# wtsi-svi/ReadServer

Hardware: AMD Instinct MI355X
Metric: 31-mer backward-search queries/sec on popBWT, counted as (query x shard) backward searches/s (higher is better)
Workload: dtype u64

## Files before the change

### include/rsbwt.h

```cpp
#ifndef RSBWT_H
#define RSBWT_H

#include <stddef.h>
#include <stdint.h>

#ifdef __cplusplus
extern "C" {
#endif

#define RSBWT_OK 0
#define RSBWT_EINVAL (-1)
#define RSBWT_EIO (-2)
#define RSBWT_EFORMAT (-3)
#define RSBWT_ENOMEM (-4)
#define RSBWT_ENODEV (-5)
#define RSBWT_EHIP (-6)
#define RSBWT_ERANGE (-7)
#define RSBWT_ESYS (-8)

#define RSBWT_OPEN_READS 1u
#define RSBWT_OPEN_KTAB_GROUPED 2u
#define RSBWT_KTAB_SHIFT 5
#define RSBWT_KTAB_MASK (0x1Fu << RSBWT_KTAB_SHIFT)
#define RSBWT_KTAB_NONE (31u << RSBWT_KTAB_SHIFT)
// ... 99 lines not shown
size_t rsbwt_1mm_scratch_bytes(const rsbwt_t *h, size_t m, uint32_t k);
int rsbwt_find_intervals_1mm_dev(rsbwt_t *h, const void *d_packed, const void *d_valid, size_t m, uint32_t k,
                                 void *d_lower, void *d_upper, void *d_scratch, void *stream);
size_t rsbwt_hits_1mm_scratch_bytes(const rsbwt_t *h, size_t m, uint32_t k);
int rsbwt_hits_1mm_dev(rsbwt_t *h, const void *d_packed, const void *d_valid, size_t m, uint32_t k, void *d_hits,
                       size_t cap, void *d_total, void *d_scratch, void *stream);
int rsbwt_extract_dev(rsbwt_t *h, const void *d_rows, size_t n, void *d_out, uint32_t stride, void *d_len,
                      void *d_prefix_len, void *stream);

int rsbwt_last_search_ms(rsbwt_t *h, float *ms);
int rsbwt_search_history_ms(rsbwt_t *h, float *ms, size_t cap, size_t *count);
int rsbwt_set_counting(rsbwt_t *h, int on);
int rsbwt_last_search_work(rsbwt_t *h, uint64_t *lf_steps, uint64_t *occ_lookups,
                           uint64_t *line_reads);
int rsbwt_last_search_counters(rsbwt_t *h, uint64_t *words16);
int rsbwt_last_search_ktab_lookups(rsbwt_t *h, uint64_t *lookups);
int rsbwt_last_search_phases(rsbwt_t *h, uint64_t *cycles6, uint64_t *passes);

#define RSBWT_SYNTH_LONG_RUNS (1ull << 63)
int rsbwt_synth_runs_dev(void *d_runs, uint64_t num_runs, uint64_t seed, int device, void *stream);
int rsbwt_synth_runs_host(uint8_t *runs, uint64_t num_runs, uint64_t seed);
int rsbwt_synth_runs_dev_at(void *d_runs, uint64_t first, uint64_t num_runs, uint64_t seed, int device, void *stream);
int rsbwt_sample_present_kmers_dev(rsbwt_t *h, size_t Q, uint32_t k, size_t stride, uint64_t seed,
                                   void *d_kmers, void *stream);
int rsbwt_synth_popbwt(const char *bwt_path, const char *reads_path, uint64_t seed,
                       uint64_t genome_len, uint32_t haplotypes, double snp_rate,
                       uint32_t read_len, double coverage, int shard, int num_shards);

int rsbwt_bpi2_write(const char *bwt_path, const char *bpi2_path);
int rsbwt_bpi2_check(rsbwt_t *h, const char *bpi2_path, uint64_t max_samples, uint64_t *checked,
// ... 189 lines not shown
                                size_t cap_rows, void *d_strings, void *d_copies, void *d_matches, void *d_carriers, void *d_status8,
                                void *stream);
int rsbwt_sample_keys(const uint8_t *codes, size_t C, uint32_t size_of_sample, uint64_t *keys);
void rsbwt_set_sample_last_work(uint64_t *work6);
uint64_t rsbwt_set_meta_head_bytes(const rsbwt_set_t *s);
size_t rsbwt_set_hits_1mm_scratch_bytes(const rsbwt_set_t *s, size_t m, uint32_t k);
int rsbwt_set_hits_1mm_is_fused(const rsbwt_set_t *s, size_t m, uint32_t k);
int rsbwt_set_hits_1mm_dev(rsbwt_set_t *s, const void *d_packed, const void *d_valid, size_t m, uint32_t k, void *d_hits,
                           size_t cap_per_shard, void *d_totals, void *d_scratch, void *stream);
int rsbwt_set_extract_dev(rsbwt_set_t *s, const void *d_rows, size_t n, void *d_out, uint32_t stride, void *d_len,
                          void *d_prefix_len, void *stream);
int rsbwt_rccl_available(void);
int rsbwt_set_set_counting(rsbwt_set_t *s, int on);
int rsbwt_set_search_history_ms(rsbwt_set_t *s, float *ms, size_t cap, size_t *count);
int rsbwt_set_last_search_counters(rsbwt_set_t *s, uint64_t *words16);

int rsbwt_service_counts(rsbwt_set_t *set, const uint8_t *requests, size_t requests_len, const uint64_t *req_off,
                         size_t n, uint8_t *replies, size_t cap, uint64_t *rep_off, size_t *needed);
int rsbwt_proto_decode_request(const uint8_t *msg, size_t len, int *t, int *rt, const char **q, size_t *qlen);
size_t rsbwt_proto_encode_count_reply(uint8_t *out, size_t cap, int request_type, const char *q, size_t qlen,
                                      int revcomp, int32_t c);
size_t rsbwt_proto_encode_reads_reply(uint8_t *out, size_t cap, int request_type, const char *q, size_t qlen, int revcomp,
                                      const char *const *reads, const size_t *read_len, size_t nreads);

size_t rsbwt_proto_encode_kmer_reply(uint8_t *out, size_t cap, int return_type, const char *q, size_t qlen, int revcomp,
                                     const char *const *reads, const size_t *read_len, size_t nreads);
int rsbwt_proto_decode_request_ks(const uint8_t *msg, size_t len, int32_t *k, int *has_k, int32_t *s, int *has_s);
size_t rsbwt_proto_encode_empty_reply(uint8_t *out, size_t cap, int t, int rt, const char *q, size_t qlen, int revcomp);

size_t rsbwt_proto_encode_all_reply(uint8_t *out, size_t cap, int request_type, int return_type, const char *q, size_t qlen, int revcomp,
// ... 81 lines not shown
```

### readserver_amd/_native.py

```python
import ctypes as C
import os
import subprocess
import threading

_HERE = os.path.dirname(os.path.abspath(__file__))
_LIB = os.environ.get("RSBWT_LIB") or os.path.join(_HERE, "lib", "librsbwt.so")
_lock = threading.Lock()
_lib = None

RSBWT_OK = 0
RSBWT_ENODEV = -5


class RsbwtError(RuntimeError):
    def __init__(self, code, msg):
        super().__init__(f"rsbwt error {code}: {msg}")
        self.code = code


def lib_path():
    return _LIB


def build(force=False):
# ... 68 lines not shown
    "rsbwt_packed_pairs_bytes": (C.c_size_t, [C.c_size_t]),
    "rsbwt_pack_interval_pairs_dev": (C.c_int, [_vp, C.c_size_t, _vp, _vp, C.c_int, _vp]),
    "rsbwt_unpack_interval_pairs_dev": (C.c_int, [_vp, C.c_size_t, _vp, C.c_int, _vp]),
    "rsbwt_pack_reads_dev": (C.c_int, [_vp, _vp, C.c_size_t, C.c_uint32, _vp, C.c_int, _vp]),
    "rsbwt_unpack_reads_dev": (C.c_int, [_vp, _vp, C.c_size_t, C.c_uint32, _vp, C.c_int, _vp]),
    "rsbwt_hits_1mm_scratch_bytes": (C.c_size_t, [_vp, C.c_size_t, C.c_uint32]),
    "rsbwt_hits_1mm_dev": (C.c_int, [_vp, _vp, _vp, C.c_size_t, C.c_uint32, _vp, C.c_size_t, _vp, _vp, _vp]),
    "rsbwt_set_1mm_scratch_bytes": (C.c_size_t, [_vp, C.c_size_t, C.c_uint32]),
    "rsbwt_set_find_intervals_1mm_dev": (C.c_int, [_vp, _vp, _vp, C.c_size_t, C.c_uint32, _vp, _vp, _vp, _vp]),
    "rsbwt_extract_dev": (C.c_int, [_vp, _vp, C.c_size_t, _vp, C.c_uint32, _vp, _vp, _vp]),
    "rsbwt_last_search_ms": (C.c_int, [_vp, C.POINTER(C.c_float)]),
    "rsbwt_search_history_ms": (C.c_int, [_vp, C.POINTER(C.c_float), C.c_size_t, C.POINTER(C.c_size_t)]),
    "rsbwt_set_counting": (C.c_int, [_vp, C.c_int]),
    "rsbwt_last_search_work": (C.c_int, [_vp, _u64p, _u64p, _u64p]),
    "rsbwt_last_search_counters": (C.c_int, [_vp, _u64p]),
    "rsbwt_last_search_phases": (C.c_int, [_vp, _u64p, _u64p]),
    "rsbwt_last_search_ktab_lookups": (C.c_int, [_vp, _u64p]),
    "rsbwt_synth_runs_dev": (C.c_int, [_vp, C.c_uint64, C.c_uint64, C.c_int, _vp]),
    "rsbwt_synth_runs_dev_at": (C.c_int, [_vp, C.c_uint64, C.c_uint64, C.c_uint64, C.c_int, _vp]),
    "rsbwt_synth_runs_host": (C.c_int, [_vp, C.c_uint64, C.c_uint64]),
    "rsbwt_sample_present_kmers_dev": (C.c_int, [_vp, C.c_size_t, C.c_uint32, C.c_size_t, C.c_uint64, _vp, _vp]),
    "rsbwt_bpi2_write": (C.c_int, [C.c_char_p, C.c_char_p]),
    "rsbwt_bpi2_check": (C.c_int, [C.c_void_p, C.c_char_p, C.c_uint64, C.POINTER(C.c_uint64), C.POINTER(C.c_uint64)]),
    "rsbwt_bpi2_validate_file": (C.c_int, [C.c_char_p]),
    "rsbwt_synth_popbwt": (C.c_int, [C.c_char_p, C.c_char_p, C.c_uint64, C.c_uint64, C.c_uint32, C.c_double,
                                     C.c_uint32, C.c_double, C.c_int, C.c_int]),
    "rsbwt_service_counts": (C.c_int, [_vp, _vp, C.c_size_t, _vp, C.c_size_t, _vp, C.c_size_t, _vp, C.POINTER(C.c_size_t)]),
    "rsbwt_service_config_load": (C.c_int, [C.c_char_p, C.POINTER(_vp)]),
    "rsbwt_service_config_free": (None, [_vp]),
    "rsbwt_service_config_get": (C.c_char_p, [_vp, C.c_char_p]),
# ... 124 lines not shown
    "rsbwt_proto_decode_request_ks": (C.c_int, [_vp, C.c_size_t, C.POINTER(C.c_int32), C.POINTER(C.c_int), C.POINTER(C.c_int32),
                                                C.POINTER(C.c_int)]),
    "rsbwt_service_set_kmermatch": (C.c_int, [_vp, C.c_int]),
    "rsbwt_service_set_unserved": (None, [_vp, C.c_int]),
    "rsbwt_set_hits_1mm_scratch_bytes": (C.c_size_t, [_vp, C.c_size_t, C.c_uint32]),
    "rsbwt_set_hits_1mm_is_fused": (C.c_int, [_vp, C.c_size_t, C.c_uint32]),
    "rsbwt_set_hits_1mm_dev": (C.c_int, [_vp, _vp, _vp, C.c_size_t, C.c_uint32, _vp, C.c_size_t, _vp, _vp, _vp]),
    "rsbwt_set_extract_dev": (C.c_int, [_vp, _vp, C.c_size_t, _vp, C.c_uint32, _vp, _vp, _vp]),
    "rsbwt_set_records_bytes": (C.c_size_t, [_vp, C.c_size_t]),
    "rsbwt_set_prepare_dev": (C.c_int, [_vp, _vp, _vp, C.c_size_t, C.c_uint32, _vp, _vp]),
    "rsbwt_set_find_interval_pairs_prepared_dev": (C.c_int, [_vp, _vp, _vp, _vp, C.c_size_t, C.c_uint32, _vp, _vp]),
    "rsbwt_rccl_available": (C.c_int, []),
    "rsbwt_set_set_counting": (C.c_int, [_vp, C.c_int]),
    "rsbwt_set_search_history_ms": (C.c_int, [_vp, C.POINTER(C.c_float), C.c_size_t, C.POINTER(C.c_size_t)]),
    "rsbwt_set_last_search_counters": (C.c_int, [_vp, _u64p]),
    "rsbwt_layout_selftest_host": (C.c_int, [_vp, C.c_uint64, C.c_uint32, _u64p, _u64p]),
    "rsbwt_layout_selftest_psi_host": (C.c_int, [_vp, C.c_uint64, C.c_uint32, _u64p, _u64p]),
    "rsbwt_layout_lines_host": (C.c_int, [_vp, C.c_uint64, C.c_uint32, C.c_uint32, _vp, C.c_uint64, _vp, C.c_uint64, _vp, C.c_uint64, _vp]),
    "rsbwt_ktab_group_selftest_host": (C.c_int, [_vp, _vp, C.c_size_t, _vp]),
    "rsbwt_debug_fast_window": (C.c_int, [_vp, C.c_size_t, C.c_uint32, _vp, _vp, C.c_int]),
    "rsbwt_debug_poke": (C.c_int, [_vp, C.c_int, C.c_uint64, _vp, C.c_size_t]),
    "rsbwt_debug_dollar_count": (C.c_int, [_vp, _vp, C.c_size_t, _vp, _vp]),
    "rsbwt_debug_rank_primitives": (C.c_int, [C.c_uint32, C.c_int, _vp, C.c_size_t, _vp, C.c_int]),
    "rsbwt_debug_staged_rank": (C.c_int, [_vp, _vp, C.c_size_t, _vp]),
    "rsbwt_set_shard": (_vp, [_vp, C.c_size_t]),
    "rsbwt_set_find_intervals": (C.c_int, [_vp, _vp, C.c_size_t, C.c_uint32, C.c_size_t, _vp, _vp]),
    "rsbwt_set_count": (C.c_int, [_vp, _vp, C.c_size_t, C.c_uint32, C.c_size_t, _vp]),
}


# ... 28 lines not shown
```

### readserver_amd/csrc/capi.hip

```cpp
#include <hip/hip_runtime.h>
#include <stdarg.h>
#include <stdio.h>
#include <stdlib.h>
#include <string.h>

#include <algorithm>
#include <condition_variable>
#include <mutex>
#include <new>
#include <string>
#include <vector>

#include "../../include/rsbwt.h"
#include "bpi2.h"
#include "bwt_file.h"
#include "capi_guard.h"
#include "capi_internal.h"
#include "kernels.h"
#include "line_format.h"

using namespace rsb;

namespace rsb {

// ... 1741 lines not shown
    if (!h) return fail(RSBWT_EINVAL, "null handle");
    int rc = use_device(h->device);
    if (rc) return rc;
    uint64_t w[WORK_WORDS];
    if ((rc = meter_work(*h, w, WORK_WORDS)) != RSBWT_OK) return rc;
    if (lf_steps) *lf_steps = w[0];
    if (occ_lookups) *occ_lookups = w[1];
    if (line_reads) *line_reads = w[2];
    return RSBWT_OK;
}

int rsbwt_last_search_counters(rsbwt_t *h, uint64_t *words16) {
    if (!h || !words16) return fail(RSBWT_EINVAL, "null argument");
    int rc = use_device(h->device);
    if (rc) return rc;
    return meter_work(*h, words16, WORK_WORDS);
}

int rsbwt_last_search_phases(rsbwt_t *h, uint64_t *cycles, uint64_t *passes) {
    if (!h || !cycles || !passes) return fail(RSBWT_EINVAL, "null argument");
    int rc = use_device(h->device);
    if (rc) return rc;
    uint64_t w[WORK_WORDS];
    if ((rc = meter_work(*h, w, WORK_WORDS)) != RSBWT_OK) return rc;
    for (int i = 0; i < 6; ++i) cycles[i] = w[4 + i];
    *passes = w[10];
    return RSBWT_OK;
}

int rsbwt_last_search_ktab_lookups(rsbwt_t *h, uint64_t *lookups) {
    if (!h || !lookups) return fail(RSBWT_EINVAL, "null argument");
// ... 383 lines not shown
```

### readserver_amd/csrc/extract_lines.hip

```cpp
#include <hip/hip_runtime.h>
#include <stdint.h>
#include <stdlib.h>

#include "kernels.h"
#include "line_format.h"
#include "rank_device.h"
#include "wave_lines.h"

namespace rsb {

#ifndef RSB_WALK_WG_WAVES
#define RSB_WALK_WG_WAVES 4
#endif
#ifndef RSB_WALK_MIN_WGS
#define RSB_WALK_MIN_WGS 4
#endif
constexpr int XWG_WAVES = RSB_WALK_WG_WAVES;


constexpr uint32_t ROW_CHUNK = 256;
struct row_pool {
    uint64_t next = 0, end = 0;
    bool drained = false;
};
// ... 10 lines not shown
        rp.end = c + chunk < n ? c + chunk : n;
        if (c >= n) {
            rp.drained = true;
            rp.next = rp.end = 0;
        }
    }
    const uint64_t mine = rp.next + __builtin_popcountll(mask & ((1ull << lane) - 1ull));
    const bool got = want && mine < rp.end;
    if (got) *row = (size_t)mine;
    const uint64_t taken = rp.next + __builtin_popcountll(mask);
    rp.next = taken < rp.end ? taken : rp.end;
    return got;
}

enum { XW_PASSES = 0, XW_ACTIVE = 1, XW_STEPS = 2, XW_CONT = 3, XW_FETCHED = 4, XW_CYCLES = 5, XW_WAIT = 6, XW_PROBES = 7, XW_WORDS = 8 };

template <bool COUNT_WORK, bool RAGGED = false>
__global__ void __launch_bounds__(64 * XWG_WAVES, RSB_WALK_MIN_WGS)
extract_prefix_wave_kernel(const shard_view *__restrict__ shards, uint32_t nshards, const uint64_t *__restrict__ rows_all,
                           size_t n_padded, uint8_t *__restrict__ out_all, uint32_t stride, uint32_t *__restrict__ plen_all,
                           unsigned long long *__restrict__ pools, unsigned long long *__restrict__ work, uint32_t row_chunk,
                           const uint64_t *__restrict__ seg = nullptr, size_t seg_stride = 0) {
    __shared__ uint4 s_stage[XWG_WAVES][64 * SLOT_U4];
    const uint32_t lane = threadIdx.x & 63u, wave = threadIdx.x >> 6;
    uint4 *stage = s_stage[wave];
    const uint32_t stage_lds = __builtin_amdgcn_readfirstlane((uint32_t)(uintptr_t)(lds_void_ptr)stage);
    const staged_line L = {own_stage_row(stage, lane), lane & 7u};
    unsigned long long xw[XW_WORDS] = {0, 0, 0, 0, 0, 0, 0, 0};
    const unsigned long long t_begin = COUNT_WORK ? __builtin_amdgcn_s_memtime() : 0ull;
    uint32_t sid = blockIdx.x % nshards;
    for (uint32_t visited = 0; visited < nshards; ++visited, sid = (sid + 1u == nshards) ? 0u : sid + 1u) {
    const shard_view *sv = shards + sid;
    const char *lines_bytes = reinterpret_cast<const char *>(sv->lines);
    const uint32_t S = sv->sp.S, nlines = (uint32_t)sv->nlines;
    const double inv = sv->sp.inv;
    const uint64_t ix_n = sv->n;
    const size_t base = RAGGED ? (size_t)seg[(size_t)sid * seg_stride] : (size_t)sid * n_padded;
    const size_t n = RAGGED ? (size_t)seg[((size_t)sid + 1u) * seg_stride] - base : n_padded;
    const uint64_t *__restrict__ rows = rows_all + base;
    uint8_t *__restrict__ out = out_all + base * stride;
    uint32_t *__restrict__ plen = plen_all + base;
    unsigned long long *pool = pools + (size_t)sid * POOL_STRIDE;
    uint32_t ctab_lo, ctab_hi;
    {
        const uint64_t c1 = sv->C[1], c2 = sv->C[2], c3 = sv->C[3], c4 = sv->C[4];
        const uint32_t l3 = lane & 3u;
        const uint64_t cv = l3 == 0u ? c1 : l3 == 1u ? c2 : l3 == 2u ? c3 : c4;
        ctab_lo = (uint32_t)cv;
        ctab_hi = (uint32_t)(cv >> 32);
    }
    bool have = false;
    row_pool rp;
    uint32_t r = 0;
    uint64_t idx = 0;
    uint32_t len = 0;
    uint32_t cont = 0, cblk = 0, cdw = 0, co = 0, tries = 0, w = 0;
    uint32_t acc_lo[4] = {0, 0, 0, 0}, acc_hi = 0;
    const bool packed_out = (stride & 3u) == 0u && ((uintptr_t)out & 3u) == 0u;
    const bool out16 = (stride & 15u) == 0u && ((uintptr_t)out & 15u) == 0u;
    uint32_t chars = 0, q1 = 0, q2 = 0, q3 = 0;
    for (;;) {
        size_t nr = 0;
        if (draw_row(!have, pool, n, lane, rp, &nr, row_chunk)) {
            r = (uint32_t)nr;
            idx = rows[r];
            len = 0;
            cont = 0;
            chars = 0;
            q1 = q2 = q3 = 0;
            have = true;
            if (idx >= ix_n) {
                plen[r] = 0xFFFFFFFFu;
                have = false;
            }
        }
        if (__builtin_amdgcn_ballot_w64(have) == 0ull) {
            if (rp.drained) break;
            continue;
        }
        if (COUNT_WORK) {
            ++xw[XW_PASSES];
            xw[XW_ACTIVE] += __builtin_popcountll(__builtin_amdgcn_ballot_w64(have));
            xw[XW_CONT] += __builtin_popcountll(__builtin_amdgcn_ballot_w64(have && cont != 0u));
        }
// ... 62 lines not shown
        const uint32_t c = cr.c;
        const uint32_t ci = (c - 1u) & 3u;
        uint64_t base;
        if (in_chunk) {
            const uint2 hd = L.u2(cdw);
            const uint32_t hw = ci < 2u ? hd.x : hd.y;
            const uint32_t alo = ci == 0u ? acc_lo[0] : ci == 1u ? acc_lo[1] : ci == 2u ? acc_lo[2] : acc_lo[3];
            base = (((uint64_t)((acc_hi >> (8u * ci)) & 0xFFu) << 32) | alo) + ((hw >> (12u * (ci & 1u))) & 0xFFFu);
        } else {
            const uint32_t hb = read_half(L, ci + 1u);
            const uint32_t m = matched24(L, HDR_DWORDS + 6u * (cq & 2u), cr.tab);
            base = read_count(L, ci + 1u) + (cq >= 2u ? hb : 0u) + ((cq & 1u) ? m : 0u);
        }
        const uint64_t pc = ((uint64_t)(uint32_t)__builtin_amdgcn_ds_bpermute((int)(ci << 2), (int)ctab_hi) << 32) |
                            (uint32_t)__builtin_amdgcn_ds_bpermute((int)(ci << 2), (int)ctab_lo);
        bool done = false;
        if (scan) {
            if (c == 0u || c > 4u) {
                if (out16) {
                    const uint32_t rem = len & 15u, nd = rem >> 2, sh = rem & 3u;
                    uint8_t *row = out + r * (size_t)stride;
                    const uint32_t B = stride - (len - rem);
                    for (uint32_t jj = 0; jj < nd; ++jj) {
                        const uint32_t di = nd - 1u - jj;
                        const uint32_t lo_d = di == 0u ? chars : di == 1u ? q1 : q2;
                        const uint32_t hi_d = di == 0u ? q1 : di == 1u ? q2 : q3;
                        const uint32_t v = sh == 0u ? lo_d : sh == 1u ? __builtin_amdgcn_alignbyte(hi_d, lo_d, 1u)
                                                   : sh == 2u ? __builtin_amdgcn_alignbyte(hi_d, lo_d, 2u)
                                                              : __builtin_amdgcn_alignbyte(hi_d, lo_d, 3u);
                        *reinterpret_cast<uint32_t *>(row + B - 4u * (jj + 1u)) = v;
                    }
                    for (uint32_t t = 0; t < sh; ++t) row[stride - len + t] = (uint8_t)(chars >> (8u * t));
                } else if (packed_out) {
                    for (uint32_t t = 0; t < (len & 3u); ++t)
                        out[r * (size_t)stride + (stride - len + t)] = (uint8_t)(chars >> (8u * t));
                }
                plen[r] = len;
                have = false;
            } else if (len == stride) {
                plen[r] = 0xFFFFFFFFu;
                have = false;
            } else {
                const uint32_t ch = (0x54474341u >> (8u * ci)) & 0xFFu;
                if (out16) {
                    q3 = __builtin_amdgcn_alignbyte(q3, q2, 3u);
                    q2 = __builtin_amdgcn_alignbyte(q2, q1, 3u);
                    q1 = __builtin_amdgcn_alignbyte(q1, chars, 3u);
                    chars = (chars << 8) | ch;
                    if ((len & 15u) == 15u)
                        *reinterpret_cast<uint4 *>(out + r * (size_t)stride + (stride - 1u - len)) = make_uint4(chars, q1, q2, q3);
                } else if (packed_out) {
                    chars = (chars << 8) | ch;
                    if ((len & 3u) == 3u) {
                        *reinterpret_cast<uint32_t *>(out + r * (size_t)stride + (stride - 1u - len)) = chars;
                    }
                } else {
                    out[r * (size_t)stride + (stride - 1u - len)] = (uint8_t)ch;
                }
                ++len;
                idx = pc + base + cr.occ - 1ull;
                cont = 0;
                done = true;
            }
        }
        if (COUNT_WORK) xw[XW_STEPS] += __builtin_popcountll(__builtin_amdgcn_ballot_w64(done));
    }
    }
    if (COUNT_WORK && lane == 0u) {
        xw[XW_CYCLES] = __builtin_amdgcn_s_memtime() - t_begin;
        for (int i = 0; i < XW_WORDS; ++i) atomicAdd(&work[i], xw[i]);
    }
}

template <bool COUNT_WORK, bool RAGGED = false>
__global__ void __launch_bounds__(64 * XWG_WAVES, RSB_WALK_MIN_WGS)
extract_postfix_wave_kernel(const shard_view *__restrict__ shards, uint32_t nshards, const uint64_t *__restrict__ rows_all,
                            size_t n_padded, uint8_t *__restrict__ out_all, uint32_t stride, const uint32_t *__restrict__ plen_all,
                            uint32_t *__restrict__ tlen_all, unsigned long long *__restrict__ pools,
                            unsigned long long *__restrict__ work, uint32_t row_chunk, const uint64_t *__restrict__ seg = nullptr,
                            size_t seg_stride = 0) {
    __shared__ uint4 s_stage[XWG_WAVES][64 * SLOT_U4];
    const uint32_t lane = threadIdx.x & 63u, wave = threadIdx.x >> 6;
    uint4 *stage = s_stage[wave];
    const uint32_t stage_lds = __builtin_amdgcn_readfirstlane((uint32_t)(uintptr_t)(lds_void_ptr)stage);
    const staged_line L = {own_stage_row(stage, lane), lane & 7u};
// ... 305 lines not shown
                }
                fresh = false;
                hv = false;
            }
        }
        if (COUNT_WORK) xw[XW_PROBES] += __builtin_popcountll(__builtin_amdgcn_ballot_w64(hinted_now));
    }
    }
    if (COUNT_WORK && lane == 0u) {
        xw[XW_CYCLES] = __builtin_amdgcn_s_memtime() - t_begin;
        for (int i = 0; i < XW_WORDS; ++i) atomicAdd(&work[i], xw[i]);
    }
}

__global__ void __launch_bounds__(256)
move_prefix16_kernel(uint8_t *__restrict__ out, uint32_t stride, const uint32_t *__restrict__ plen, size_t n) {
    const size_t r = ((size_t)blockIdx.x * blockDim.x + threadIdx.x) >> 4;
    const uint32_t sub = threadIdx.x & 15u;
    uint32_t pl = r < n ? plen[r] : 0u;
    if (pl == 0xFFFFFFFFu || pl >= stride) pl = 0u;
    uint8_t *buf = out + (r < n ? r : 0) * (size_t)stride;
    const uint32_t off = stride - pl;
    for (uint32_t k0 = 0; __builtin_amdgcn_ballot_w64(k0 < pl) != 0ull; k0 += 256u) {
        const uint32_t k = k0 + 16u * sub;
        const bool active = k < pl;
        uint4 A = make_uint4(0, 0, 0, 0), B = make_uint4(0, 0, 0, 0);
        uint32_t sh = 0;
        if (active) {
            const uint32_t a = off + k, a0 = a & ~15u;
            sh = a & 15u;
            A = *reinterpret_cast<const uint4 *>(buf + a0);
            if (a0 + 16u < stride) B = *reinterpret_cast<const uint4 *>(buf + a0 + 16u);
        }
        __builtin_amdgcn_s_waitcnt(0x0F70);
// ... 23 lines not shown
    const uint32_t off = stride - pl;
    for (uint32_t k0 = 0; k0 < pl; k0 += 64u) {
        const uint32_t k = k0 + lane;
        uint8_t ch = 0;
        if (k < pl) ch = buf[off + k];
        __builtin_amdgcn_s_waitcnt(0x0F70);
        __builtin_amdgcn_wave_barrier();
        if (k < pl) buf[k] = ch;
    }
}

static size_t extract_wgs_per_cu() {
    static const size_t v = (size_t)knob_int("RSBWT_EXTRACT_WGS_PER_CU", 1, 20, RSB_WALK_MIN_WGS);
    return v;
}

template <bool RAGGED, bool CW>
static hipError_t launch_walks(scratch_cache &scratch, const shard_view *d_shards, uint32_t nshards, const uint64_t *rows, size_t n, size_t total,
                               const uint64_t *seg, size_t seg_stride, uint8_t *out, uint32_t stride, uint32_t *plen, uint32_t *len, int num_cus,
                               hipStream_t stream, unsigned long long *d_work) {
    pool_lease mem(scratch, stream, 0, 2, nshards);
    if (mem.error() != hipSuccess) return mem.error();
    const size_t g = plan_grid(total, 64 * XWG_WAVES, resident_cap(num_cus, extract_wgs_per_cu()), nshards);
    const uint32_t row_chunk = plan_draw(ROW_CHUNK, 1, g * XWG_WAVES, 2, total);
    hipLaunchKernelGGL((extract_prefix_wave_kernel<CW, RAGGED>), dim3((unsigned)g), dim3(64 * XWG_WAVES), 0, stream, d_shards, nshards, rows, n, out,
                       stride, plen, mem.pool(0, nshards), d_work, row_chunk, seg, seg_stride);
    if ((stride & 15u) == 0u && ((uintptr_t)out & 15u) == 0u)
        hipLaunchKernelGGL(move_prefix16_kernel, dim3((unsigned)((total + 15) / 16)), dim3(256), 0, stream, out, stride, (const uint32_t *)plen, total);
    else
        hipLaunchKernelGGL(move_prefix_kernel, dim3((unsigned)((total + 3) / 4)), dim3(256), 0, stream, out, stride, (const uint32_t *)plen, total);
    hipLaunchKernelGGL((extract_postfix_wave_kernel<CW, RAGGED>), dim3((unsigned)g), dim3(64 * XWG_WAVES), 0, stream, d_shards, nshards, rows, n, out,
                       stride, (const uint32_t *)plen, len, mem.pool(1, nshards), CW ? d_work + XW_WORDS : nullptr, row_chunk, seg, seg_stride);
    return hipGetLastError();
}

hipError_t launch_extract_wave(scratch_cache &scratch, const shard_view *d_shards, uint32_t nshards, const void *d_rows,
                               size_t n, void *d_out, uint32_t stride, void *d_plen, void *d_len, int num_cus,
                               hipStream_t stream, unsigned long long *d_work) {
    if (n == 0 || nshards == 0) return hipSuccess;
    constexpr size_t MAX_ROWS = 1ull << 31;
    if (n > MAX_ROWS) {
        if (nshards != 1) return hipErrorInvalidValue;
        for (size_t i0 = 0; i0 < n; i0 += MAX_ROWS) {
            const size_t m = n - i0 < MAX_ROWS ? n - i0 : MAX_ROWS;
            const hipError_t e2 = launch_extract_wave(scratch, d_shards, 1, (const uint64_t *)d_rows + i0, m, (uint8_t *)d_out + i0 * (size_t)stride,
                                                      stride, (uint32_t *)d_plen + i0, (uint32_t *)d_len + i0, num_cus, stream, d_work);
            if (e2 != hipSuccess) return e2;
        }
        return hipSuccess;
    }
    const auto walks = d_work ? launch_walks<false, true> : launch_walks<false, false>;
    return walks(scratch, d_shards, nshards, (const uint64_t *)d_rows, n, n * (size_t)nshards, nullptr, 0, (uint8_t *)d_out, stride, (uint32_t *)d_plen,
                 (uint32_t *)d_len, num_cus, stream, d_work);
}

hipError_t launch_extract_ragged(scratch_cache &scratch, const shard_view *d_shards, uint32_t nshards, const void *d_rows, size_t total,
                                 const void *d_seg, size_t seg_stride, void *d_out, uint32_t stride, void *d_plen, void *d_len, int num_cus,
                                 hipStream_t stream) {
    if (total == 0 || nshards == 0) return hipSuccess;
    if (total >= (1ull << 31) || !d_seg) return hipErrorInvalidValue;
    return launch_walks<true, false>(scratch, d_shards, nshards, (const uint64_t *)d_rows, 0, total, (const uint64_t *)d_seg, seg_stride,
                                     (uint8_t *)d_out, stride, (uint32_t *)d_plen, (uint32_t *)d_len, num_cus, stream, nullptr);
}

}
```

### readserver_amd/csrc/kernels.h

```cpp
#ifndef RSBWT_KERNELS_H
#define RSBWT_KERNELS_H

#include <hip/hip_runtime.h>
#include <stddef.h>
#include <stdint.h>

#include <mutex>

#include "launch_plan.h"
#include "line_format.h"

namespace rsb {

class scratch_cache {
  public:
    struct lease {
        void *p = nullptr;
        int slot = -1;
    };
    hipError_t take(size_t bytes, hipStream_t stream, lease *out);
    void give(const lease &l, hipStream_t stream);
    void destroy();
    size_t held_bytes();

// ... 2 lines not shown
    struct slot_t {
        void *p = nullptr;
        size_t bytes = 0;
        hipStream_t last = nullptr;
        hipEvent_t done = nullptr;
        bool recorded = false, busy = false;
    };
    slot_t slots_[SLOTS];
    std::mutex mu_;
};

constexpr uint32_t POOL_STRIDE = 32;

class pool_lease {
  public:
    pool_lease(scratch_cache &scratch, hipStream_t stream, size_t front_bytes, uint32_t npools, uint32_t nshards)
        : scratch_(scratch), stream_(stream) {
        const size_t pool_bytes = (size_t)npools * nshards * POOL_STRIDE * sizeof(unsigned long long);
        err_ = scratch.take(front_bytes + pool_bytes, stream, &mem_);
        if (err_ != hipSuccess) return;
        pools_ = (unsigned long long *)((char *)mem_.p + front_bytes);
        err_ = hipMemsetAsync(pools_, 0, pool_bytes, stream);
    }
    ~pool_lease() { scratch_.give(mem_, stream_); }
    pool_lease(const pool_lease &) = delete;
    pool_lease &operator=(const pool_lease &) = delete;
    hipError_t error() const { return err_; }
    void *front() const { return mem_.p; }
    unsigned long long *pool(uint32_t i, uint32_t nshards) const { return pools_ + (size_t)i * nshards * POOL_STRIDE; }

  private:
    scratch_cache &scratch_;
    hipStream_t stream_;
    scratch_cache::lease mem_;
    unsigned long long *pools_ = nullptr;
    hipError_t err_;
};

hipError_t launch_pack(const void *d_kmers, size_t Q, uint32_t k, size_t stride, void *d_packed,
                       void *d_valid, hipStream_t stream);

__host__ __device__ inline size_t hit_map_words(size_t Q) { return ((Q + 127) / 128) * 2; }

struct search_extra {
    void *d_trace_out = nullptr;
    const void *d_trace_in = nullptr;
    uint32_t trace_n = 0, variants = 0;
    bool table_build = false;
    bool pairs = false;
    void *d_hit_bits = nullptr;
// ... 60 lines not shown
constexpr uint32_t WL_COUNT_STRIDE = 32;
hipError_t launch_mm1_worklists(const shard_view *d_shards, uint32_t nshards, const void *d_packed, const void *d_valid, size_t m,
                                uint32_t k, uint32_t tn, const void *d_trace, const void *d_own, void *d_worklists, size_t wl_cap,
                                void *d_counts, void *d_sparse, void *d_hit_bits, int num_cus, hipStream_t stream,
                                unsigned long long *d_branch_work = nullptr);
hipError_t launch_search_worklist(scratch_cache &scratch, const shard_view *d_shards, uint32_t nshards, const void *d_packed,
                                  const void *d_valid, size_t m, uint32_t tn, const void *d_worklists, const void *d_counts, size_t wl_cap,
                                  uint32_t k, void *d_sparse, void *d_hit_bits, unsigned long long *d_work, int num_cus,
                                  hipStream_t stream, hipEvent_t ev0 = nullptr, hipEvent_t ev1 = nullptr, const void *d_pre = nullptr);
hipError_t launch_wl_table_entries(const shard_view *d_shards, uint32_t nshards, const void *d_packed, size_t m, uint32_t k, uint32_t tn,
                                   void *d_pre, hipStream_t stream);
hipError_t launch_search_walk(scratch_cache &scratch, const shard_view *d_shards, uint32_t nshards, const void *d_packed,
                              const void *d_valid, size_t m, uint32_t tn, void *d_worklists, void *d_counts, size_t wl_cap, uint32_t k,
                              void *d_sparse, void *d_hit_bits, unsigned long long *d_work, int num_cus, hipStream_t stream,
                              hipEvent_t ev0 = nullptr, hipEvent_t ev1 = nullptr);
constexpr int WORK_WORDS = 16;

hipError_t build_ktable(const shard_view &view, uint32_t T, uint64_t *d_entries, uint32_t stride, int num_cus,
                        hipStream_t stream, uint32_t fmt = KTAB_PLAIN, uint64_t *untabulated = nullptr);

hipError_t launch_occ_batch(const shard_view &ix, const void *d_syms, const void *d_index, size_t n,
                            void *d_out, hipStream_t stream);
hipError_t launch_char_batch(const shard_view &ix, const void *d_index, size_t n, void *d_out,
                             hipStream_t stream);
hipError_t launch_occ_at_batch(const shard_view &ix, const void *d_syms, const void *d_bc, size_t n, void *d_out,
                               hipStream_t stream);
size_t compact_hits_block_words(size_t n_searches);
hipError_t launch_compact_hits(const void *d_bits, const void *d_sparse, size_t n_searches, void *d_hits, size_t cap,
                               void *d_total, void *d_block_counts, hipStream_t stream, uint32_t nseg = 1);
hipError_t launch_pack_pairs10(const void *d_pairs, size_t n, void *d_packed, void *d_unfit, hipStream_t stream);
hipError_t launch_unpack_pairs10(const void *d_packed, size_t n, void *d_pairs, hipStream_t stream);
hipError_t launch_pack_reads2(const void *d_reads, const void *d_len, size_t n, uint32_t stride, void *d_packed, hipStream_t stream);
hipError_t launch_unpack_reads2(const void *d_packed, const void *d_len, size_t n, uint32_t stride, void *d_reads, hipStream_t stream);
hipError_t launch_variants(const void *d_packed, const void *d_valid, size_t Q, uint32_t k, void *d_vpacked,
                           void *d_vvalid, hipStream_t stream);
hipError_t launch_debug_fast_window(const void *d_p, size_t n, uint32_t S, void *d_w, void *d_r, hipStream_t stream);
uint64_t select_sample_stride(const shard_view &ix);
hipError_t launch_select_samples(const shard_view &ix, uint64_t *d_sel, hipStream_t stream);
hipError_t launch_psi_hints(const shard_view &ix, unsigned long long *d_made, hipStream_t stream);
hipError_t launch_extract_wave(scratch_cache &scratch, const shard_view *d_shards, uint32_t nshards, const void *d_rows,
                               size_t n, void *d_out, uint32_t stride, void *d_plen, void *d_len, int num_cus,
                               hipStream_t stream, unsigned long long *d_work = nullptr);
hipError_t launch_extract_ragged(scratch_cache &scratch, const shard_view *d_shards, uint32_t nshards, const void *d_rows, size_t total,
                                 const void *d_seg, size_t seg_stride, void *d_out, uint32_t stride, void *d_plen, void *d_len, int num_cus,
                                 hipStream_t stream);
hipError_t launch_locate(scratch_cache &scratch, const shard_view *d_shards, uint32_t nshards, const void *d_shard_of, const void *d_rows,
                         size_t n, uint32_t max_steps, void *d_read_row, void *d_ordinal, void *d_offset, unsigned long long *d_work2,
                         int num_cus, hipStream_t stream);
size_t interval_rows_scan_bytes(size_t n);
hipError_t launch_interval_totals(const shard_view *d_views, uint32_t S, const void *d_pairs, size_t Q, uint64_t max_rows, void *d_matches,
                                  void *d_kept, void *d_first, void *d_over, void *d_temp, size_t temp_bytes, hipStream_t stream);
hipError_t launch_interval_cells(const shard_view *d_views, uint32_t S, const void *d_pairs, size_t Q, uint64_t max_rows, const void *d_matches,
                                 void *d_cellw, void *d_cellpos, void *d_temp, size_t temp_bytes, hipStream_t stream);
hipError_t launch_interval_fill(const shard_view *d_views, uint32_t S, const void *d_pairs, size_t Q, const void *d_first, size_t cap,
                                void *d_shard, void *d_rows, const void *d_cellpos, void *d_cell_rows, void *d_dest, hipStream_t stream);
struct gt_batch {
    const char *text;
    const uint32_t *nprev;
    const uint64_t *q_off;
    const uint32_t *q_len;
// ... 94 lines not shown
```

### readserver_amd/csrc/sets.hip

```cpp
#include <dlfcn.h>
#include <hip/hip_runtime.h>
#include <rccl/rccl.h>
#include <stdint.h>
#include <stdio.h>
#include <stdlib.h>
#include <string.h>

#include <algorithm>
#include <atomic>
#include <new>
#include <string>
#include <thread>
#include <unordered_set>
#include <utility>
#include <vector>

#include "../../include/rsbwt.h"
#include "capi_guard.h"
#include "capi_internal.h"
#include "meta_file.h"
#include "sample_codes.h"
#include "service.h"

using namespace rsb;
// ... 1165 lines not shown
    if (total > cap_reads) return fail(RSBWT_ERANGE, "%llu reads over the set, room for %zu", (unsigned long long)total, cap_reads);
    if (total == 0) return RSBWT_OK;
    if (!reads || !read_len) return fail(RSBWT_EINVAL, "null argument");
    if (total >= (1ull << 31)) return CAPPED_TAKE_HOST;
    uint8_t *d_cellw = ci.d_extra, *d_cellpos = d_cellw + a_cells;
    hipError_t e = launch_interval_cells(g->d_views, S, ci.d_pairs, Q, max_rows, ci.d_matches, d_cellw, d_cellpos, ci.d_tmp, ci.tmp_bytes, st);
    if (e != hipSuccess) return fail_hip(e, "interval-rows kernels");
    if ((rc = ensure_group_xviews(s, g, st)) != RSBWT_OK) return rc;
    const size_t a_rows = al256(total * 8), a_u32 = al256(total * 4), a_out = al256(total * (size_t)read_stride);
    e = g->scratch.take(a_rows + 4 * a_u32 + a_out, st, &gc.lb);
    if (e != hipSuccess) return fail(RSBWT_ENOMEM, "%llu reads of %u bytes do not fit the device's free memory: %s", (unsigned long long)total,
                                     read_stride, hipGetErrorString(e));
    uint8_t *d_crow = (uint8_t *)gc.lb.p, *d_out = d_crow + a_rows, *d_dest = d_out + a_out, *d_shard = d_dest + a_u32, *d_plen = d_shard + a_u32,
            *d_rlen = d_plen + a_u32;
    e = launch_interval_fill(g->d_views, S, ci.d_pairs, Q, ci.d_first, (size_t)total, d_shard, nullptr, d_cellpos, d_crow, d_dest, st);
    if (e == hipSuccess)
        e = launch_extract_ragged(g->scratch, g->d_xviews, S, d_crow, (size_t)total, d_cellpos, Q, d_out, read_stride, d_plen, d_rlen, g->num_cus, st);
    if (e != hipSuccess) return fail_hip(e, "row expansion and extract kernel launches");
    capped_last_work[0] = total;
    std::vector<char> ho(total * (size_t)read_stride);
    std::vector<uint32_t> hl(total), hd(total), hs(total);
    HIP_OK(hipMemcpyAsync(ho.data(), d_out, total * (size_t)read_stride, hipMemcpyDeviceToHost, st));
    HIP_OK(hipMemcpyAsync(hl.data(), d_rlen, total * 4, hipMemcpyDeviceToHost, st));
    HIP_OK(hipMemcpyAsync(hd.data(), d_dest, total * 4, hipMemcpyDeviceToHost, st));
    HIP_OK(hipMemcpyAsync(hs.data(), d_shard, total * 4, hipMemcpyDeviceToHost, st));
    HIP_OK(hipStreamSynchronize(st));
    for (size_t t = 0; t < total; ++t) {
        scatter_read(ho.data(), hl.data(), nullptr, hd[t], reads, read_stride, read_len, nullptr, t);
        if (read_shard) read_shard[t] = (uint32_t)g->idx[hs[t]];
    }
    return RSBWT_OK;
}
// ... 2158 lines not shown
    }
    return RSBWT_OK;
}

int rsbwt_set_search_history_ms(rsbwt_set_t *s, float *ms, size_t cap, size_t *count) {
    if (!s || (!ms && cap) || !count) return fail(RSBWT_EINVAL, "null argument");
    int rc = use_device(s->groups[0]->device);
    if (rc) return rc;
    return meter_history_ms(*s->groups[0], ms, cap, count);
}

int rsbwt_set_last_search_counters(rsbwt_set_t *s, uint64_t *words16) {
    if (!s || !words16) return fail(RSBWT_EINVAL, "null argument");
    int rc = use_device(s->groups[0]->device);
    if (rc) return rc;
    return meter_work(*s->groups[0], words16, WORK_WORDS);
}

}
```

Baseline: 4.428 billion.

## Buffer extracted prefixes in registers and store in place, skipping the move pass

The prefix extract walk now packs bases 2-bit into a register array of up to 256 characters. When a read ends, the wave writes it directly to its final position at the start of the output row. Only reads longer than the cap spill to the row tail and are flagged in a bitmap, so the move kernel shifts only those rows. This targets the extra global read and write of every prefix by the move pass, and adds register pressure, a per-flush readlane loop, and a bitmap memset. The benchmark measures k-mer backward search, which this extract path probably does not touch.

```diff
diff --git a/include/rsbwt.h b/include/rsbwt.h
--- a/include/rsbwt.h
+++ b/include/rsbwt.h
@@ -137,6 +137,7 @@
 int rsbwt_last_search_work(rsbwt_t *h, uint64_t *lf_steps, uint64_t *occ_lookups,
                            uint64_t *line_reads);
 int rsbwt_last_search_counters(rsbwt_t *h, uint64_t *words16);
+int rsbwt_last_extract_stores(rsbwt_t *h, uint64_t *in_place, uint64_t *moved);
 int rsbwt_last_search_ktab_lookups(rsbwt_t *h, uint64_t *lookups);
 int rsbwt_last_search_phases(rsbwt_t *h, uint64_t *cycles6, uint64_t *passes);
 
@@ -356,6 +357,7 @@
 int rsbwt_set_set_counting(rsbwt_set_t *s, int on);
 int rsbwt_set_search_history_ms(rsbwt_set_t *s, float *ms, size_t cap, size_t *count);
 int rsbwt_set_last_search_counters(rsbwt_set_t *s, uint64_t *words16);
+int rsbwt_set_last_extract_stores(rsbwt_set_t *s, uint64_t *in_place, uint64_t *moved);
 
 int rsbwt_service_counts(rsbwt_set_t *set, const uint8_t *requests, size_t requests_len, const uint64_t *req_off,
                          size_t n, uint8_t *replies, size_t cap, uint64_t *rep_off, size_t *needed);
diff --git a/readserver_amd/_native.py b/readserver_amd/_native.py
--- a/readserver_amd/_native.py
+++ b/readserver_amd/_native.py
@@ -106,6 +106,7 @@
     "rsbwt_set_counting": (C.c_int, [_vp, C.c_int]),
     "rsbwt_last_search_work": (C.c_int, [_vp, _u64p, _u64p, _u64p]),
     "rsbwt_last_search_counters": (C.c_int, [_vp, _u64p]),
+    "rsbwt_last_extract_stores": (C.c_int, [_vp, _u64p, _u64p]),
     "rsbwt_last_search_phases": (C.c_int, [_vp, _u64p, _u64p]),
     "rsbwt_last_search_ktab_lookups": (C.c_int, [_vp, _u64p]),
     "rsbwt_synth_runs_dev": (C.c_int, [_vp, C.c_uint64, C.c_uint64, C.c_int, _vp]),
@@ -260,6 +261,7 @@
     "rsbwt_set_set_counting": (C.c_int, [_vp, C.c_int]),
     "rsbwt_set_search_history_ms": (C.c_int, [_vp, C.POINTER(C.c_float), C.c_size_t, C.POINTER(C.c_size_t)]),
     "rsbwt_set_last_search_counters": (C.c_int, [_vp, _u64p]),
+    "rsbwt_set_last_extract_stores": (C.c_int, [_vp, _u64p, _u64p]),
     "rsbwt_layout_selftest_host": (C.c_int, [_vp, C.c_uint64, C.c_uint32, _u64p, _u64p]),
     "rsbwt_layout_selftest_psi_host": (C.c_int, [_vp, C.c_uint64, C.c_uint32, _u64p, _u64p]),
     "rsbwt_layout_lines_host": (C.c_int, [_vp, C.c_uint64, C.c_uint32, C.c_uint32, _vp, C.c_uint64, _vp, C.c_uint64, _vp, C.c_uint64, _vp]),
diff --git a/readserver_amd/csrc/base_pack.h b/readserver_amd/csrc/base_pack.h
--- /dev/null
+++ b/readserver_amd/csrc/base_pack.h
@@ -0,0 +1,66 @@
+#ifndef RSBWT_BASE_PACK_H
+#define RSBWT_BASE_PACK_H
+
+#include <stdint.h>
+
+#if defined(__HIPCC__)
+#define RSB_PACK_FN __host__ __device__ __forceinline__
+#define RSB_PACK_UNROLL _Pragma("unroll")
+#else
+#define RSB_PACK_FN inline
+#define RSB_PACK_UNROLL
+#endif
+
+namespace rsb {
+
+#ifndef RSB_PFX_CAP
+#define RSB_PFX_CAP 256
+#endif
+constexpr uint32_t PFX_CAP = RSB_PFX_CAP;
+constexpr int PFX_WORDS = (int)(PFX_CAP / 16u);
+static_assert(PFX_CAP % 16u == 0u && PFX_WORDS >= 4, "whole 16-base chunks; the walk's fallback keeps 16 characters in four of the words");
+
+constexpr uint32_t BASE_ASCII = 0x54474341u;
+
+template <int W>
+RSB_PACK_FN void pack_push_front(uint32_t (&w)[W], uint32_t code) {
+    RSB_PACK_UNROLL
+    for (int i = W - 1; i > 0; --i) w[i] = (w[i] << 2) | (w[i - 1] >> 30);
+    w[0] = (w[0] << 2) | (code & 3u);
+}
+
+template <int W>
+RSB_PACK_FN uint32_t pack_word(const uint32_t (&w)[W], uint32_t c) {
+    uint32_t v = 0;
+    RSB_PACK_UNROLL
+    for (int i = 0; i < W; ++i) v = c == (uint32_t)i ? w[i] : v;
+    return v;
+}
+
+template <int W>
+RSB_PACK_FN uint32_t pack_chunk(const uint32_t (&w)[W], uint32_t off, uint32_t c) {
+    const uint32_t here = pack_word(w, c);
+    if (off == 0u) return here;
+    const uint32_t below = c == 0u ? 0u : pack_word(w, c - 1u);
+    return (here << (2u * off)) | (below >> (32u - 2u * off));
+}
+
+RSB_PACK_FN uint32_t pack_expand4(uint32_t codes8) {
+    uint32_t s = codes8 & 0xFFu;
+    s = (s | (s << 12)) & 0x000F000Fu;
+    s = (s | (s << 6)) & 0x03030303u;
+#if defined(__HIP_DEVICE_COMPILE__)
+    return __builtin_amdgcn_perm(BASE_ASCII, BASE_ASCII, s);
+#else
+    uint32_t v = 0;
+    for (int k = 0; k < 4; ++k) v |= ((BASE_ASCII >> (8u * ((s >> (8 * k)) & 3u))) & 0xFFu) << (8 * k);
+    return v;
+#endif
+}
+RSB_PACK_FN void pack_expand16(uint32_t codes, uint32_t (&out)[4]) {
+    RSB_PACK_UNROLL
+    for (int d = 0; d < 4; ++d) out[d] = pack_expand4(codes >> (8 * d));
+}
+
+}
+#endif
diff --git a/readserver_amd/csrc/capi.hip b/readserver_amd/csrc/capi.hip
--- a/readserver_amd/csrc/capi.hip
+++ b/readserver_amd/csrc/capi.hip
@@ -1779,7 +1779,18 @@
     if (!h || !words16) return fail(RSBWT_EINVAL, "null argument");
     int rc = use_device(h->device);
     if (rc) return rc;
-    return meter_work(*h, words16, WORK_WORDS);
+    return meter_work(*h, words16, WORK_WORDS_PUBLIC);
+}
+
+int rsbwt_last_extract_stores(rsbwt_t *h, uint64_t *in_place, uint64_t *moved) {
+    if (!h || !in_place || !moved) return fail(RSBWT_EINVAL, "null argument");
+    int rc = use_device(h->device);
+    if (rc) return rc;
+    uint64_t w[WORK_WORDS];
+    if ((rc = meter_work(*h, w, WORK_WORDS)) != RSBWT_OK) return rc;
+    *in_place = w[WORK_WORDS_PUBLIC];
+    *moved = w[WORK_WORDS_PUBLIC + 1];
+    return RSBWT_OK;
 }
 
 int rsbwt_last_search_phases(rsbwt_t *h, uint64_t *cycles, uint64_t *passes) {
diff --git a/readserver_amd/csrc/extract_lines.hip b/readserver_amd/csrc/extract_lines.hip
--- a/readserver_amd/csrc/extract_lines.hip
+++ b/readserver_amd/csrc/extract_lines.hip
@@ -2,6 +2,7 @@
 #include <stdint.h>
 #include <stdlib.h>
 
+#include "base_pack.h"
 #include "kernels.h"
 #include "line_format.h"
 #include "rank_device.h"
@@ -48,20 +49,24 @@
 }
 
 enum { XW_PASSES = 0, XW_ACTIVE = 1, XW_STEPS = 2, XW_CONT = 3, XW_FETCHED = 4, XW_CYCLES = 5, XW_WAIT = 6, XW_PROBES = 7, XW_WORDS = 8 };
+enum { XW_INPLACE = 2 * XW_WORDS, XW_MOVED = 2 * XW_WORDS + 1 };
+static_assert(XW_MOVED < WORK_WORDS, "the counters of a counting launch (kernels.h)");
 
 template <bool COUNT_WORK, bool RAGGED = false>
 __global__ void __launch_bounds__(64 * XWG_WAVES, RSB_WALK_MIN_WGS)
 extract_prefix_wave_kernel(const shard_view *__restrict__ shards, uint32_t nshards, const uint64_t *__restrict__ rows_all,
                            size_t n_padded, uint8_t *__restrict__ out_all, uint32_t stride, uint32_t *__restrict__ plen_all,
                            unsigned long long *__restrict__ pools, unsigned long long *__restrict__ work, uint32_t row_chunk,
-                           const uint64_t *__restrict__ seg = nullptr, size_t seg_stride = 0) {
+                           uint32_t *__restrict__ moved_bits, const uint64_t *__restrict__ seg = nullptr, size_t seg_stride = 0) {
     __shared__ uint4 s_stage[XWG_WAVES][64 * SLOT_U4];
     const uint32_t lane = threadIdx.x & 63u, wave = threadIdx.x >> 6;
     uint4 *stage = s_stage[wave];
     const uint32_t stage_lds = __builtin_amdgcn_readfirstlane((uint32_t)(uintptr_t)(lds_void_ptr)stage);
     const staged_line L = {own_stage_row(stage, lane), lane & 7u};
     unsigned long long xw[XW_WORDS] = {0, 0, 0, 0, 0, 0, 0, 0};
+    unsigned long long x_inplace = 0, x_moved = 0;
     const unsigned long long t_begin = COUNT_WORK ? __builtin_amdgcn_s_memtime() : 0ull;
+    const bool in_place = moved_bits != nullptr;
     uint32_t sid = blockIdx.x % nshards;
     for (uint32_t visited = 0; visited < nshards; ++visited, sid = (sid + 1u == nshards) ? 0u : sid + 1u) {
     const shard_view *sv = shards + sid;
@@ -92,7 +97,9 @@
     uint32_t acc_lo[4] = {0, 0, 0, 0}, acc_hi = 0;
     const bool packed_out = (stride & 3u) == 0u && ((uintptr_t)out & 3u) == 0u;
     const bool out16 = (stride & 15u) == 0u && ((uintptr_t)out & 15u) == 0u;
-    uint32_t chars = 0, q1 = 0, q2 = 0, q3 = 0;
+    uint32_t pk[PFX_WORDS] = {};
+    uint32_t &chars = pk[0], &q1 = pk[1], &q2 = pk[2], &q3 = pk[3];
+    const size_t row0 = base;
     for (;;) {
         size_t nr = 0;
         if (draw_row(!have, pool, n, lane, rp, &nr, row_chunk)) {
@@ -100,8 +107,6 @@
             idx = rows[r];
             len = 0;
             cont = 0;
-            chars = 0;
-            q1 = q2 = q3 = 0;
             have = true;
             if (idx >= ix_n) {
                 plen[r] = 0xFFFFFFFFu;
@@ -194,10 +199,13 @@
         }
         const uint64_t pc = ((uint64_t)(uint32_t)__builtin_amdgcn_ds_bpermute((int)(ci << 2), (int)ctab_hi) << 32) |
                             (uint32_t)__builtin_amdgcn_ds_bpermute((int)(ci << 2), (int)ctab_lo);
-        bool done = false;
+        bool done = false, flush = false, ended = false;
         if (scan) {
             if (c == 0u || c > 4u) {
-                if (out16) {
+                ended = true;
+                if (in_place && len <= PFX_CAP) {
+                    flush = true;
+                } else if (out16) {
                     const uint32_t rem = len & 15u, nd = rem >> 2, sh = rem & 3u;
                     uint8_t *row = out + r * (size_t)stride;
                     const uint32_t B = stride - (len - rem);
@@ -221,8 +229,21 @@
                 plen[r] = 0xFFFFFFFFu;
                 have = false;
             } else {
-                const uint32_t ch = (0x54474341u >> (8u * ci)) & 0xFFu;
-                if (out16) {
+                const uint32_t ch = (BASE_ASCII >> (8u * ci)) & 0xFFu;
+                if (in_place && len == PFX_CAP) {
+                    uint8_t *at = out + r * (size_t)stride + (stride - PFX_CAP);
+#pragma unroll
+                    for (int j = 0; j < PFX_WORDS; ++j) {
+                        uint32_t a[4];
+                        pack_expand16(pk[j], a);
+                        *reinterpret_cast<uint4 *>(at + 16 * j) = make_uint4(a[0], a[1], a[2], a[3]);
+                    }
+                    const size_t g = row0 + r;
+                    atomicOr(moved_bits + (g >> 5), 1u << (g & 31u));
+                }
+                if (in_place && len < PFX_CAP) {
+                    pack_push_front(pk, ci);
+                } else if (out16) {
                     q3 = __builtin_amdgcn_alignbyte(q3, q2, 3u);
                     q2 = __builtin_amdgcn_alignbyte(q2, q1, 3u);
                     q1 = __builtin_amdgcn_alignbyte(q1, chars, 3u);
@@ -243,12 +264,34 @@
                 done = true;
             }
         }
-        if (COUNT_WORK) xw[XW_STEPS] += __builtin_popcountll(__builtin_amdgcn_ballot_w64(done));
+        if (in_place) {
+            uint64_t fm = __builtin_amdgcn_ballot_w64(flush);
+            if (COUNT_WORK) x_inplace += __builtin_popcountll(fm);
+            while (fm != 0ull) {
+                const int src = __builtin_ctzll(fm);
+                fm &= fm - 1ull;
+                const uint32_t fr = (uint32_t)__builtin_amdgcn_readlane((int)r, src), fl = (uint32_t)__builtin_amdgcn_readlane((int)len, src);
+                uint32_t uw[PFX_WORDS];
+#pragma unroll
+                for (int i = 0; i < PFX_WORDS; ++i) uw[i] = (uint32_t)__builtin_amdgcn_readlane((int)pk[i], src);
+                if (16u * lane < fl) {
+                    uint32_t a[4];
+                    pack_expand16(pack_chunk(uw, 0u, lane), a);
+                    *reinterpret_cast<uint4 *>(out + fr * (size_t)stride + 16u * lane) = make_uint4(a[0], a[1], a[2], a[3]);
+                }
+            }
+        }
+        if (COUNT_WORK) {
+            xw[XW_STEPS] += __builtin_popcountll(__builtin_amdgcn_ballot_w64(done));
+            x_moved += __builtin_popcountll(__builtin_amdgcn_ballot_w64(ended && !flush));
+        }
     }
     }
     if (COUNT_WORK && lane == 0u) {
         xw[XW_CYCLES] = __builtin_amdgcn_s_memtime() - t_begin;
         for (int i = 0; i < XW_WORDS; ++i) atomicAdd(&work[i], xw[i]);
+        atomicAdd(&work[XW_INPLACE], x_inplace);
+        atomicAdd(&work[XW_MOVED], x_moved);
     }
 }
 
@@ -584,10 +627,12 @@
 }
 
 __global__ void __launch_bounds__(256)
-move_prefix16_kernel(uint8_t *__restrict__ out, uint32_t stride, const uint32_t *__restrict__ plen, size_t n) {
+move_prefix16_kernel(uint8_t *__restrict__ out, uint32_t stride, const uint32_t *__restrict__ plen, size_t n,
+                     const uint32_t *__restrict__ moved_bits) {
     const size_t r = ((size_t)blockIdx.x * blockDim.x + threadIdx.x) >> 4;
     const uint32_t sub = threadIdx.x & 15u;
-    uint32_t pl = r < n ? plen[r] : 0u;
+    const bool mine = r < n && (moved_bits == nullptr || ((moved_bits[r >> 5] >> (r & 31u)) & 1u) != 0u);
+    uint32_t pl = mine ? plen[r] : 0u;
     if (pl == 0xFFFFFFFFu || pl >= stride) pl = 0u;
     uint8_t *buf = out + (r < n ? r : 0) * (size_t)stride;
     const uint32_t off = stride - pl;
@@ -641,19 +686,27 @@
     static const size_t v = (size_t)knob_int("RSBWT_EXTRACT_WGS_PER_CU", 1, 20, RSB_WALK_MIN_WGS);
     return v;
 }
+static bool extract_legacy_prefix() {
+    static const bool v = knob_set("RSBWT_EXTRACT_LEGACY_PREFIX");
+    return v;
+}
 
 template <bool RAGGED, bool CW>
 static hipError_t launch_walks(scratch_cache &scratch, const shard_view *d_shards, uint32_t nshards, const uint64_t *rows, size_t n, size_t total,
                                const uint64_t *seg, size_t seg_stride, uint8_t *out, uint32_t stride, uint32_t *plen, uint32_t *len, int num_cus,
                                hipStream_t stream, unsigned long long *d_work) {
-    pool_lease mem(scratch, stream, 0, 2, nshards);
+    const bool aligned16 = (stride & 15u) == 0u && ((uintptr_t)out & 15u) == 0u;
+    const bool in_place = aligned16 && !extract_legacy_prefix();
+    pool_lease mem(scratch, stream, 0, 2, nshards, in_place ? (total + 31) / 32 * sizeof(uint32_t) : 0);
     if (mem.error() != hipSuccess) return mem.error();
+    uint32_t *moved_bits = (uint32_t *)mem.tail();
     const size_t g = plan_grid(total, 64 * XWG_WAVES, resident_cap(num_cus, extract_wgs_per_cu()), nshards);
     const uint32_t row_chunk = plan_draw(ROW_CHUNK, 1, g * XWG_WAVES, 2, total);
     hipLaunchKernelGGL((extract_prefix_wave_kernel<CW, RAGGED>), dim3((unsigned)g), dim3(64 * XWG_WAVES), 0, stream, d_shards, nshards, rows, n, out,
-                       stride, plen, mem.pool(0, nshards), d_work, row_chunk, seg, seg_stride);
-    if ((stride & 15u) == 0u && ((uintptr_t)out & 15u) == 0u)
-        hipLaunchKernelGGL(move_prefix16_kernel, dim3((unsigned)((total + 15) / 16)), dim3(256), 0, stream, out, stride, (const uint32_t *)plen, total);
+                       stride, plen, mem.pool(0, nshards), d_work, row_chunk, moved_bits, seg, seg_stride);
+    if (aligned16)
+        hipLaunchKernelGGL(move_prefix16_kernel, dim3((unsigned)((total + 15) / 16)), dim3(256), 0, stream, out, stride, (const uint32_t *)plen, total,
+                           (const uint32_t *)moved_bits);
     else
         hipLaunchKernelGGL(move_prefix_kernel, dim3((unsigned)((total + 3) / 4)), dim3(256), 0, stream, out, stride, (const uint32_t *)plen, total);
     hipLaunchKernelGGL((extract_postfix_wave_kernel<CW, RAGGED>), dim3((unsigned)g), dim3(64 * XWG_WAVES), 0, stream, d_shards, nshards, rows, n, out,
@@ -683,11 +736,12 @@
 
 hipError_t launch_extract_ragged(scratch_cache &scratch, const shard_view *d_shards, uint32_t nshards, const void *d_rows, size_t total,
                                  const void *d_seg, size_t seg_stride, void *d_out, uint32_t stride, void *d_plen, void *d_len, int num_cus,
-                                 hipStream_t stream) {
+                                 hipStream_t stream, unsigned long long *d_work) {
     if (total == 0 || nshards == 0) return hipSuccess;
     if (total >= (1ull << 31) || !d_seg) return hipErrorInvalidValue;
-    return launch_walks<true, false>(scratch, d_shards, nshards, (const uint64_t *)d_rows, 0, total, (const uint64_t *)d_seg, seg_stride,
-                                     (uint8_t *)d_out, stride, (uint32_t *)d_plen, (uint32_t *)d_len, num_cus, stream, nullptr);
-}
-
-}
+    const auto walks = d_work ? launch_walks<true, true> : launch_walks<true, false>;
+    return walks(scratch, d_shards, nshards, (const uint64_t *)d_rows, 0, total, (const uint64_t *)d_seg, seg_stride, (uint8_t *)d_out, stride,
+                 (uint32_t *)d_plen, (uint32_t *)d_len, num_cus, stream, d_work);
+}
+
+}
diff --git a/readserver_amd/csrc/kernels.h b/readserver_amd/csrc/kernels.h
--- a/readserver_amd/csrc/kernels.h
+++ b/readserver_amd/csrc/kernels.h
@@ -40,13 +40,14 @@
 
 class pool_lease {
   public:
-    pool_lease(scratch_cache &scratch, hipStream_t stream, size_t front_bytes, uint32_t npools, uint32_t nshards)
+    pool_lease(scratch_cache &scratch, hipStream_t stream, size_t front_bytes, uint32_t npools, uint32_t nshards, size_t tail_bytes = 0)
         : scratch_(scratch), stream_(stream) {
         const size_t pool_bytes = (size_t)npools * nshards * POOL_STRIDE * sizeof(unsigned long long);
-        err_ = scratch.take(front_bytes + pool_bytes, stream, &mem_);
+        err_ = scratch.take(front_bytes + pool_bytes + tail_bytes, stream, &mem_);
         if (err_ != hipSuccess) return;
         pools_ = (unsigned long long *)((char *)mem_.p + front_bytes);
-        err_ = hipMemsetAsync(pools_, 0, pool_bytes, stream);
+        tail_ = tail_bytes ? (char *)pools_ + pool_bytes : nullptr;
+        err_ = hipMemsetAsync(pools_, 0, pool_bytes + tail_bytes, stream);
     }
     ~pool_lease() { scratch_.give(mem_, stream_); }
     pool_lease(const pool_lease &) = delete;
@@ -54,12 +55,14 @@
     hipError_t error() const { return err_; }
     void *front() const { return mem_.p; }
     unsigned long long *pool(uint32_t i, uint32_t nshards) const { return pools_ + (size_t)i * nshards * POOL_STRIDE; }
+    void *tail() const { return tail_; }
 
   private:
     scratch_cache &scratch_;
     hipStream_t stream_;
     scratch_cache::lease mem_;
     unsigned long long *pools_ = nullptr;
+    void *tail_ = nullptr;
     hipError_t err_;
 };
 
@@ -150,7 +153,8 @@
                               const void *d_valid, size_t m, uint32_t tn, void *d_worklists, void *d_counts, size_t wl_cap, uint32_t k,
                               void *d_sparse, void *d_hit_bits, unsigned long long *d_work, int num_cus, hipStream_t stream,
                               hipEvent_t ev0 = nullptr, hipEvent_t ev1 = nullptr);
-constexpr int WORK_WORDS = 16;
+constexpr int WORK_WORDS_PUBLIC = 16;
+constexpr int WORK_WORDS = 18;
 
 hipError_t build_ktable(const shard_view &view, uint32_t T, uint64_t *d_entries, uint32_t stride, int num_cus,
                         hipStream_t stream, uint32_t fmt = KTAB_PLAIN, uint64_t *untabulated = nullptr);
@@ -179,7 +183,7 @@
                                hipStream_t stream, unsigned long long *d_work = nullptr);
 hipError_t launch_extract_ragged(scratch_cache &scratch, const shard_view *d_shards, uint32_t nshards, const void *d_rows, size_t total,
                                  const void *d_seg, size_t seg_stride, void *d_out, uint32_t stride, void *d_plen, void *d_len, int num_cus,
-                                 hipStream_t stream);
+                                 hipStream_t stream, unsigned long long *d_work = nullptr);
 hipError_t launch_locate(scratch_cache &scratch, const shard_view *d_shards, uint32_t nshards, const void *d_shard_of, const void *d_rows,
                          size_t n, uint32_t max_steps, void *d_read_row, void *d_ordinal, void *d_offset, unsigned long long *d_work2,
                          int num_cus, hipStream_t stream);
diff --git a/readserver_amd/csrc/sets.hip b/readserver_amd/csrc/sets.hip
--- a/readserver_amd/csrc/sets.hip
+++ b/readserver_amd/csrc/sets.hip
@@ -1203,8 +1203,14 @@
     uint8_t *d_crow = (uint8_t *)gc.lb.p, *d_out = d_crow + a_rows, *d_dest = d_out + a_out, *d_shard = d_dest + a_u32, *d_plen = d_shard + a_u32,
             *d_rlen = d_plen + a_u32;
     e = launch_interval_fill(g->d_views, S, ci.d_pairs, Q, ci.d_first, (size_t)total, d_shard, nullptr, d_cellpos, d_crow, d_dest, st);
+    unsigned long long *work = nullptr;
+    if (g->counting) {
+        work = g->d_work;
+        HIP_OK(hipMemsetAsync(work, 0, WORK_WORDS * sizeof(unsigned long long), st));
+    }
     if (e == hipSuccess)
-        e = launch_extract_ragged(g->scratch, g->d_xviews, S, d_crow, (size_t)total, d_cellpos, Q, d_out, read_stride, d_plen, d_rlen, g->num_cus, st);
+        e = launch_extract_ragged(g->scratch, g->d_xviews, S, d_crow, (size_t)total, d_cellpos, Q, d_out, read_stride, d_plen, d_rlen, g->num_cus, st,
+                                  work);
     if (e != hipSuccess) return fail_hip(e, "row expansion and extract kernel launches");
     capped_last_work[0] = total;
     std::vector<char> ho(total * (size_t)read_stride);
@@ -3393,7 +3399,18 @@
     if (!s || !words16) return fail(RSBWT_EINVAL, "null argument");
     int rc = use_device(s->groups[0]->device);
     if (rc) return rc;
-    return meter_work(*s->groups[0], words16, WORK_WORDS);
-}
-
-}
+    return meter_work(*s->groups[0], words16, WORK_WORDS_PUBLIC);
+}
+
+int rsbwt_set_last_extract_stores(rsbwt_set_t *s, uint64_t *in_place, uint64_t *moved) {
+    if (!s || !in_place || !moved) return fail(RSBWT_EINVAL, "null argument");
+    int rc = use_device(s->groups[0]->device);
+    if (rc) return rc;
+    uint64_t w[WORK_WORDS];
+    if ((rc = meter_work(*s->groups[0], w, WORK_WORDS)) != RSBWT_OK) return rc;
+    *in_place = w[WORK_WORDS_PUBLIC];
+    *moved = w[WORK_WORDS_PUBLIC + 1];
+    return RSBWT_OK;
+}
+
+}
```

Measured after the change: 4.427 billion, median of 2. Within noise of the previous version (-0.0%).
